# KrishnaswamyLab/graphtools

Hardware: NVIDIA B200
Metric: graph build points/sec (kernel+diff_op) (higher is better)
Workload: dtype f32 tensor-core select (f32 accumulate) / f64 values

## Files before the change

graphtools_b200/csrc/order.cu:

```cuda
#include "common.cuh"
#include "gtb200.h"

namespace {

constexpr int ORD_DMAX = 128;
constexpr int ORD_ASSIGN_THREADS = 128;
constexpr int ORD_CHUNK = 1024;
constexpr int LIST_UNITS = 8;

__global__ void __launch_bounds__(ORD_ASSIGN_THREADS) order_assign_kernel(const float* __restrict__ X, int64_t n, int d,
                                                                          int P, int64_t pstride,
                                                                          int32_t* __restrict__ cell) {
  extern __shared__ float4 piv4[];
  const int d4 = (d + 3) / 4;
  float* piv = reinterpret_cast<float*>(piv4);
  float* pn = piv + (size_t)P * d4 * 4;
  for (int i = threadIdx.x; i < P * d4 * 4; i += blockDim.x) {
    const int pv = i / (d4 * 4), k = i - pv * d4 * 4;
    piv[i] = k < d ? X[(int64_t)pv * pstride * d + k] : 0.f;
  }
  __syncthreads();
  for (int pv = threadIdx.x; pv < P; pv += blockDim.x) {
    float s = 0.f;
    for (int k = 0; k < d4 * 4; ++k) s = fmaf(piv[pv * d4 * 4 + k], piv[pv * d4 * 4 + k], s);
    pn[pv] = s;
  }
  __syncthreads();
  const int64_t r = (int64_t)blockIdx.x * blockDim.x + threadIdx.x;
  if (r >= n) return;
  float x[ORD_DMAX];
#pragma unroll
  for (int k = 0; k < ORD_DMAX; ++k) x[k] = k < d ? X[r * d + k] : 0.f;
  float best = gtb_inf_f();
  int bi = 0;
  for (int pv = 0; pv < P; ++pv) {
    const float4* pp = piv4 + pv * d4;
    float a0 = 0.f, a1 = 0.f;
#pragma unroll
    for (int k4 = 0; k4 < ORD_DMAX / 4; ++k4) {
      if (k4 < d4) {
        const float4 q = pp[k4];
        a0 = fmaf(x[4 * k4], q.x, a0);
        a1 = fmaf(x[4 * k4 + 1], q.y, a1);
        a0 = fmaf(x[4 * k4 + 2], q.z, a0);
        a1 = fmaf(x[4 * k4 + 3], q.w, a1);
      }
    }
    const float s = pn[pv] - 2.f * (a0 + a1);
    if (s < best) { best = s; bi = pv; }
  }
  cell[r] = bi;
}

__global__ void order_count_kernel(const int32_t* __restrict__ cell, int64_t n, int P, int32_t* __restrict__ counts) {
  extern __shared__ int32_t hist[];
  for (int p = threadIdx.x; p < P; p += blockDim.x) hist[p] = 0;
  __syncthreads();
  const int64_t r0 = (int64_t)blockIdx.x * ORD_CHUNK;
  for (int64_t r = r0 + threadIdx.x; r < n && r < r0 + ORD_CHUNK; r += blockDim.x) atomicAdd(&hist[cell[r]], 1);
  __syncthreads();
  for (int p = threadIdx.x; p < P; p += blockDim.x) counts[(int64_t)blockIdx.x * P + p] = hist[p];
}

__global__ void order_cellscan_kernel(int32_t* __restrict__ counts, int64_t nchunks, int P, int32_t* __restrict__ total) {
  const int lane = threadIdx.x & 31;
  const int p = (int)(((int64_t)blockIdx.x * blockDim.x + threadIdx.x) >> 5);
  if (p >= P) return;
  int run = 0;
  for (int64_t c0 = 0; c0 < nchunks; c0 += 32) {
    const int64_t c = c0 + lane;
    const int v = c < nchunks ? counts[c * P + p] : 0;
    int inc = v;
#pragma unroll
    for (int off = 1; off < 32; off <<= 1) {
      const int o = __shfl_up_sync(0xffffffffu, inc, off);
      if (lane >= off) inc += o;
    }
    if (c < nchunks) counts[c * P + p] = run + inc - v;
    run += __shfl_sync(0xffffffffu, inc, 31);
  }
  if (lane == 0) total[p] = run;
}

__global__ void __launch_bounds__(32) order_fill_kernel(const int32_t* __restrict__ cell, int64_t n, int P,
                                                        const int32_t* __restrict__ counts,
                                                        const int32_t* __restrict__ total, int32_t* __restrict__ perm) {
  extern __shared__ int64_t off[];
  const int lane = threadIdx.x;
  int64_t run = 0;
  for (int p0 = 0; p0 < P; p0 += 32) {
    const int p = p0 + lane;
    const int64_t v = p < P ? total[p] : 0;
    int64_t inc = v;
#pragma unroll
    for (int o = 1; o < 32; o <<= 1) {
      const int64_t u = __shfl_up_sync(0xffffffffu, inc, o);
      if (lane >= o) inc += u;
    }
    if (p < P) off[p] = run + inc - v + counts[(int64_t)blockIdx.x * P + p];
    run += __shfl_sync(0xffffffffu, inc, 31);
  }
  __syncwarp();
  const int64_t r0 = (int64_t)blockIdx.x * ORD_CHUNK;
  for (int64_t rb = r0; rb < n && rb < r0 + ORD_CHUNK; rb += 32) {
    const int64_t r = rb + lane;
    const bool ok = r < n;
    const int c = ok ? cell[r] : -1 - lane;
    const unsigned peers = __match_any_sync(0xffffffffu, c);
    const int rank = __popc(peers & ((1u << lane) - 1u));
    if (ok) perm[off[c] + rank] = (int32_t)r;
    __syncwarp();
    if (ok && rank == 0) off[c] += __popc(peers);
    __syncwarp();
  }
}

template <typename T>
__global__ void tile_geometry_kernel(const T* __restrict__ X, int64_t n, int d, const int32_t* __restrict__ perm,
                                     int64_t rows, int64_t ngroups, double* __restrict__ cent, double* __restrict__ rad) {
  constexpr int J = ORD_DMAX / 32;
  const int lane = threadIdx.x & 31;
  const int64_t g = ((int64_t)blockIdx.x * blockDim.x + threadIdx.x) >> 5;
  if (g >= ngroups) return;
  const int64_t r0 = g * rows, r1 = (r0 + rows < n) ? r0 + rows : n;
  double c[J];
#pragma unroll
  for (int j = 0; j < J; ++j) c[j] = 0.0;
#pragma unroll 8
  for (int64_t r = r0; r < r1; ++r) {
    const T* xr = X + (int64_t)perm[r] * d;
#pragma unroll
    for (int j = 0; j < J; ++j) {
      const int k = lane + 32 * j;
      if (k < d) c[j] += (double)xr[k];
    }
  }
  const double inv = r1 > r0 ? 1.0 / (double)(r1 - r0) : 0.0;
#pragma unroll
  for (int j = 0; j < J; ++j) c[j] *= inv;
  double m = 0.0;
#pragma unroll 8
  for (int64_t r = r0; r < r1; ++r) {
    const T* xr = X + (int64_t)perm[r] * d;
    double s = 0.0;
#pragma unroll
    for (int j = 0; j < J; ++j) {
      const int k = lane + 32 * j;
      if (k < d) {
        const double v = (double)xr[k] - c[j];
        s = fma(v, v, s);
      }
    }
#pragma unroll
    for (int o = 16; o > 0; o >>= 1) s += __shfl_xor_sync(0xffffffffu, s, o);
    m = fmax(m, s);
  }
#pragma unroll
  for (int j = 0; j < J; ++j) {
    const int k = lane + 32 * j;
    if (k < d) cent[(int64_t)k * ngroups + g] = c[j];
  }
  if (lane == 0) rad[g] = r1 > r0 ? __dsqrt_ru(m) : -1.0;
}

__global__ void tile_lists_count_kernel(const double* __restrict__ uc, const double* __restrict__ ur,
                                        const double* __restrict__ ub, int64_t nu, const double* __restrict__ rc,
                                        const double* __restrict__ rr, int64_t nt, int d, uint8_t* __restrict__ keep,
                                        int32_t* __restrict__ count) {
  __shared__ double cu[LIST_UNITS][ORD_DMAX];
  const int64_t u0 = (int64_t)blockIdx.y * LIST_UNITS;
  for (int i = threadIdx.x; i < LIST_UNITS * d; i += blockDim.x) {
    const int u = i / d, k = i - u * d;
    cu[u][k] = (u0 + u < nu) ? uc[(int64_t)k * nu + u0 + u] : 0.0;
  }
  __syncthreads();
  const int64_t t = (int64_t)blockIdx.x * blockDim.x + threadIdx.x;
  double s[LIST_UNITS];
#pragma unroll
  for (int u = 0; u < LIST_UNITS; ++u) s[u] = 0.0;
  if (t < nt) {
    for (int k = 0; k < d; ++k) {
      const double y = rc[(int64_t)k * nt + t];
#pragma unroll
      for (int u = 0; u < LIST_UNITS; ++u) {
        const double v = cu[u][k] - y;
        s[u] = fma(v, v, s[u]);
      }
    }
  }
  const double rt = t < nt ? rr[t] * (1.0 + 1e-12) : 0.0;
#pragma unroll
  for (int u = 0; u < LIST_UNITS; ++u) {
    const int64_t uu = u0 + u;
    bool k = false;
    if (t < nt && uu < nu && ur[uu] >= 0.0) {
      const double gap = sqrt(s[u]) * (1.0 - 1e-12) - ur[uu] * (1.0 + 1e-12) - rt;
      k = !(gap > 0.0 && gap * gap * (1.0 - 1e-12) >= ub[uu]);
    }
    if (t < nt && uu < nu) keep[uu * nt + t] = k ? 1 : 0;
    const unsigned b = __ballot_sync(0xffffffffu, k);
    if ((threadIdx.x & 31) == 0 && b) atomicAdd(&count[uu], __popc(b));
  }
}

__global__ void __launch_bounds__(256) tile_lists_fill_kernel(const uint8_t* __restrict__ keep, int64_t nt,
                                                              const int64_t* __restrict__ ptr,
                                                              int32_t* __restrict__ tiles) {
  __shared__ int wsum[8];
  const int64_t u = blockIdx.x;
  const int lane = threadIdx.x & 31, warp = threadIdx.x >> 5;
  int64_t run = ptr[u];
  for (int64_t t0 = 0; t0 < nt; t0 += 256) {
    const int64_t t = t0 + threadIdx.x;
    const bool k = t < nt && keep[u * nt + t];
    const unsigned b = __ballot_sync(0xffffffffu, k);
    if (lane == 0) wsum[warp] = __popc(b);
    __syncthreads();
    int before = 0, all = 0;
#pragma unroll
    for (int w = 0; w < 8; ++w) {
      before += (w < warp) ? wsum[w] : 0;
      all += wsum[w];
    }
    if (k) tiles[run + before + __popc(b & ((1u << lane) - 1u))] = (int32_t)t;
    run += all;
    __syncthreads();
  }
}

__global__ void unpermute_kernel(const int32_t* __restrict__ cand_p, const float* __restrict__ tau_p, int64_t nq, int S,
                                 int ntau, const int32_t* __restrict__ perm_q, const int32_t* __restrict__ perm_r,
                                 int32_t* __restrict__ cand, float* __restrict__ tau) {
  const int64_t e = (int64_t)blockIdx.x * blockDim.x + threadIdx.x;
  if (e >= nq * S) return;
  const int64_t i = e / S;
  const int s = (int)(e - i * S);
  const int64_t o = perm_q[i];
  const int32_t c = cand_p[e];
  cand[o * S + s] = c >= 0 ? perm_r[c] : c;
  if (s < ntau) tau[o * ntau + s] = tau_p[i * ntau + s];
}

}

extern "C" int gtb_order_assign(const float* X, int64_t n, int d, int P, int32_t* cell, void* stream) {
  GTB_CHECK_ARG(n > 0 && d > 0 && d <= ORD_DMAX, "bad shape (d <= 128)");
  GTB_CHECK_ARG(P >= 1 && P <= 512 && P <= n, "pivot count must be in [1, min(512, n)]");
  const size_t smem = ((size_t)P * ((d + 3) / 4) * 4 + P) * sizeof(float);
  GTB_CUDA(cudaFuncSetAttribute(order_assign_kernel, cudaFuncAttributeMaxDynamicSharedMemorySize, (int)smem));
  order_assign_kernel<<<(unsigned)gtb_cdiv(n, ORD_ASSIGN_THREADS), ORD_ASSIGN_THREADS, smem, (cudaStream_t)stream>>>(
      X, n, d, P, n / P, cell);
  GTB_CHECK_LAUNCH();
  return GTB_OK;
}

extern "C" int64_t gtb_order_ws_elems(int64_t n, int P) { return gtb_cdiv(n, ORD_CHUNK) * P + P; }

extern "C" int gtb_order_sort(const int32_t* cell, int64_t n, int P, int32_t* ws, int32_t* perm, void* stream) {
  GTB_CHECK_ARG(n > 0 && P >= 1 && P <= 512, "bad shape");
  cudaStream_t st = (cudaStream_t)stream;
  const int64_t nchunks = gtb_cdiv(n, ORD_CHUNK);
  int32_t* counts = ws;
  int32_t* total = ws + nchunks * P;
  order_count_kernel<<<(unsigned)nchunks, 256, P * sizeof(int32_t), st>>>(cell, n, P, counts);
  GTB_CHECK_LAUNCH();
  order_cellscan_kernel<<<(unsigned)gtb_cdiv(P, 8), 256, 0, st>>>(counts, nchunks, P, total);
  GTB_CHECK_LAUNCH();
  order_fill_kernel<<<(unsigned)nchunks, 32, P * sizeof(int64_t), st>>>(cell, n, P, counts, total, perm);
  GTB_CHECK_LAUNCH();
  return GTB_OK;
}

extern "C" int gtb_tile_geometry(const void* X, int64_t n, int d, int x64, const int32_t* perm, int64_t rows,
                                 int64_t ngroups, double* cent, double* rad, void* stream) {
  GTB_CHECK_ARG(n > 0 && d > 0 && d <= ORD_DMAX && rows > 0 && ngroups > 0, "bad shape (d <= 128)");
  const unsigned grid = (unsigned)gtb_cdiv(ngroups * 32, 256);
  if (x64)
    tile_geometry_kernel<double><<<grid, 256, 0, (cudaStream_t)stream>>>((const double*)X, n, d, perm, rows, ngroups,
                                                                         cent, rad);
  else
    tile_geometry_kernel<float><<<grid, 256, 0, (cudaStream_t)stream>>>((const float*)X, n, d, perm, rows, ngroups,
                                                                        cent, rad);
  GTB_CHECK_LAUNCH();
  return GTB_OK;
}

extern "C" int gtb_tile_lists_count(const double* uc, const double* ur, const double* ub, int64_t nu, const double* rc,
                                    const double* rr, int64_t nt, int d, uint8_t* keep, int32_t* count, void* stream) {
  GTB_CHECK_ARG(nu > 0 && nt > 0 && d > 0 && d <= ORD_DMAX, "bad shape (d <= 128)");
  GTB_CHECK_ARG(gtb_cdiv(nu, LIST_UNITS) < 65536, "too many units");
  cudaStream_t st = (cudaStream_t)stream;
  GTB_CUDA(cudaMemsetAsync(count, 0, nu * sizeof(int32_t), st));
  tile_lists_count_kernel<<<dim3((unsigned)gtb_cdiv(nt, 256), (unsigned)gtb_cdiv(nu, LIST_UNITS)), 256, 0, st>>>(
      uc, ur, ub, nu, rc, rr, nt, d, keep, count);
  GTB_CHECK_LAUNCH();
  return GTB_OK;
}

extern "C" int gtb_tile_lists_fill(const uint8_t* keep, int64_t nu, int64_t nt, const int64_t* ptr, int32_t* tiles,
                                   void* stream) {
  GTB_CHECK_ARG(nu > 0 && nt > 0, "bad shape");
  tile_lists_fill_kernel<<<(unsigned)nu, 256, 0, (cudaStream_t)stream>>>(keep, nt, ptr, tiles);
  GTB_CHECK_LAUNCH();
  return GTB_OK;
}

extern "C" int gtb_unpermute_candidates(const int32_t* cand_p, const float* tau_p, int64_t nq, int S, int ntau,
                                        const int32_t* perm_q, const int32_t* perm_r, int32_t* cand, float* tau,
                                        void* stream) {
  GTB_CHECK_ARG(nq > 0 && S > 0 && ntau >= 1 && ntau <= S, "bad shape");
  unpermute_kernel<<<(unsigned)gtb_cdiv(nq * S, 256), 256, 0, (cudaStream_t)stream>>>(cand_p, tau_p, nq, S, ntau,
                                                                                      perm_q, perm_r, cand, tau);
  GTB_CHECK_LAUNCH();
  return GTB_OK;
}
```

graphtools_b200/csrc/search_tc.cu:

```cuda
#include "common.cuh"
#include "gtb200.h"
#include "tc_ptx.cuh"
#include <cuda.h>
#include <cuda_bf16.h>
#include <cuda_fp16.h>

namespace {

#ifndef GTB_TC_CAP
#define GTB_TC_CAP 96
#endif
#ifndef GTB_TC_HYBRID
#define GTB_TC_HYBRID 4
#endif
constexpr int TC_M = 128, TC_N = 128, TC_CAP = GTB_TC_CAP, TC_S = 32, TC_GROUPS = 2, TC_THREADS = 64 + 128 * TC_GROUPS;
static_assert(TC_CAP % 32 == 0 && TC_CAP >= TC_S + 64 && TC_CAP <= 128, "candidate buffer: TC_S kept + two batches of 32");
constexpr float TC_BIG = 1e29f;
constexpr float TC_PAD_NORM = 1e30f;
constexpr float TC_BIG_H = 50000.f;
constexpr float TC_PAD_NORM_H = 60000.f;
constexpr float TC_H_MAXNORM = 8192.f;
constexpr int64_t TC_SPLIT_ROWS_MAX = 40 * 4 * 128;
#ifndef GTB_TC_SEED_K
#define GTB_TC_SEED_K 8
#endif
constexpr int TC_SEED_K = GTB_TC_SEED_K;

using namespace gtbptx;

struct TcParams {
  int64_t nq, nq_pad, nr, nr_pad;
  int nks;
  int64_t nrounds;
  int64_t n_qclusters, tiles_per_split;
  unsigned int* sync_ctr;
  int64_t tile_stride;
  const float* seed_tau;
  int64_t q_unit0, split_k, split_row0, split_rows;
  uint2* piece_buf; uint2* piece_meta;
  const int64_t* unit_ptr; const int32_t* unit_tiles; const int32_t* unit_order; int64_t n_units;
  const float* qn2;
  int32_t* cand_idx; uint2* cand_buf; float* tau;
  const float* lim2; int2* pairs; unsigned long long capacity; unsigned long long* counter; int32_t* rowcnt;
};

__device__ __forceinline__ uint32_t f2ord(uint32_t bits) {
  return bits ^ ((uint32_t)((int32_t)bits >> 31) | 0x80000000u);
}
__device__ __forceinline__ float ord2f(uint32_t u) {
  return __uint_as_float((u & 0x80000000u) ? (u ^ 0x80000000u) : ~u);
}

template <int LS, int CAP>
__device__ __noinline__ float compact_row(uint2* buf, int cnt, int lane) {
  constexpr int NSLOT = CAP / 32;
  constexpr unsigned long long NONE = ~0ull;
  uint2 t[NSLOT];
  unsigned long long key[NSLOT];
#pragma unroll
  for (int i = 0; i < NSLOT; ++i) {
    const int e = i * 32 + lane;
    t[i] = make_uint2(0u, 0u);
    key[i] = NONE;
    if (e < cnt) {
      t[i] = buf[e];
      key[i] = ((unsigned long long)f2ord(t[i].x) << 32) | (unsigned long long)t[i].y;
    }
  }
  unsigned long long lo = 0ull, hi = NONE, T = NONE;
  for (int iter = 0; iter < CAP + 1; ++iter) {
    unsigned m[NSLOT];
#pragma unroll
    for (int i = 0; i < NSLOT; ++i) m[i] = __ballot_sync(0xffffffffu, key[i] > lo && key[i] < hi);
    unsigned long long cand = 0ull;
    unsigned mm = 0u;
#pragma unroll
    for (int i = 0; i < NSLOT; ++i) {
      const int sl = (i + iter) % NSLOT;
      unsigned long long ks = key[0];
      unsigned ms = m[0];
#pragma unroll
      for (int q = 1; q < NSLOT; ++q) { if (sl == q) { ks = key[q]; ms = m[q]; } }
      if (mm == 0u && ms != 0u) { cand = ks; mm = ms; }
    }
    if (mm == 0u) break;
    const int src = (iter & 2) ? (31 - __clz(mm)) : (__ffs(mm) - 1);
    const unsigned long long pv = __shfl_sync(0xffffffffu, cand, src);
    int c = 0;
#pragma unroll
    for (int i = 0; i < NSLOT; ++i) c += __popc(__ballot_sync(0xffffffffu, key[i] < pv));
    if (c == LS - 1) { T = pv; break; }
    if (c >= LS) hi = pv; else lo = pv;
  }
  int base = 0;
  const unsigned lt = (1u << lane) - 1u;
#pragma unroll
  for (int i = 0; i < NSLOT; ++i) {
    const bool keep = key[i] <= T;
    const unsigned km = __ballot_sync(0xffffffffu, keep);
    if (keep) buf[base + __popc(km & lt)] = t[i];
    base += __popc(km);
  }
  return ord2f((uint32_t)(T >> 32));
}

__device__ __forceinline__ float tmin32(const uint32_t (&r)[32]) {
  float b[11];
#pragma unroll
  for (int i = 0; i < 10; ++i)
    b[i] = fminf(fminf(__uint_as_float(r[3 * i]), __uint_as_float(r[3 * i + 1])), __uint_as_float(r[3 * i + 2]));
  b[10] = fminf(__uint_as_float(r[30]), __uint_as_float(r[31]));
  const float c0 = fminf(fminf(b[0], b[1]), b[2]), c1 = fminf(fminf(b[3], b[4]), b[5]);
  const float c2 = fminf(fminf(b[6], b[7]), b[8]), c3 = fminf(b[9], b[10]);
  return fminf(fminf(fminf(c0, c1), c2), c3);
}

constexpr int TC_SYNC_EVERY = 128;

__device__ __forceinline__ void tmem_st8(uint32_t taddr, const float4& a, const float4& b) {
  asm volatile("tcgen05.st.sync.aligned.32x32b.x8.b32 [%0], {%1, %2, %3, %4, %5, %6, %7, %8};"
               ::"r"(taddr), "r"(__float_as_uint(a.x)), "r"(__float_as_uint(a.y)), "r"(__float_as_uint(a.z)),
               "r"(__float_as_uint(a.w)), "r"(__float_as_uint(b.x)), "r"(__float_as_uint(b.y)),
               "r"(__float_as_uint(b.z)), "r"(__float_as_uint(b.w))
               : "memory");
}
__device__ __forceinline__ void tc_mma_ts_pred(bool bf16, uint32_t d_tmem, uint32_t a_tmem, uint64_t bdesc,
                                               uint32_t idesc, uint32_t accumulate, uint32_t leader) {
  if (bf16) {
    asm volatile(
        "{\n .reg .pred p, q;\n setp.ne.b32 p, %4, 0;\n setp.ne.b32 q, %5, 0;\n"
        " @q tcgen05.mma.cta_group::1.kind::f16 [%0], [%1], %2, %3, p;\n}"
        ::"r"(d_tmem), "r"(a_tmem), "l"(bdesc), "r"(idesc), "r"(accumulate), "r"(leader)
        : "memory");
  } else {
    asm volatile(
        "{\n .reg .pred p, q;\n setp.ne.b32 p, %4, 0;\n setp.ne.b32 q, %5, 0;\n"
        " @q tcgen05.mma.cta_group::1.kind::tf32 [%0], [%1], %2, %3, p;\n}"
        ::"r"(d_tmem), "r"(a_tmem), "l"(bdesc), "r"(idesc), "r"(accumulate), "r"(leader)
        : "memory");
  }
}
__device__ __forceinline__ void tc_commit_pred(uint32_t bar, uint32_t leader) {
  asm volatile(
      "{\n .reg .pred q;\n setp.ne.b32 q, %1, 0;\n"
      " @q tcgen05.commit.cta_group::1.mbarrier::arrive::one.shared::cluster.b64 [%0];\n}"
      ::"r"(bar), "r"(leader)
      : "memory");
}
__device__ __forceinline__ void tc_commit_mc_pred(uint32_t bar, uint16_t mask, uint32_t leader) {
  asm volatile(
      "{\n .reg .pred q;\n setp.ne.b32 q, %2, 0;\n"
      " @q tcgen05.commit.cta_group::1.mbarrier::arrive::one.shared::cluster.multicast::cluster.b64 [%0], %1;\n}"
      ::"r"(bar), "h"(mask), "r"(leader)
      : "memory");
}

template <int MODE, int CL, int FMT, int LS, int QT, bool PIECE = false, bool WIDE = false,
          bool LISTED = false>
__global__ void __launch_bounds__(TC_THREADS, 1)
search_tc_kernel(const __grid_constant__ CUtensorMap mBh, const __grid_constant__ CUtensorMap mBht,
                 const __grid_constant__ CUtensorMap mBl, const __grid_constant__ CUtensorMap mBlt,
                 const void* __restrict__ q_hi_v, const void* __restrict__ q_lo_v, TcParams p) {
  extern __shared__ unsigned char smem_raw[];
  const uint32_t raw = smem_u32(smem_raw);
  const uint32_t base = (raw + 1023u) & ~1023u;
  unsigned char* gbase = smem_raw + (base - raw);

  constexpr bool BF16 = FMT != 0;
  constexpr int NPROD = (FMT == 3) ? 1 : (FMT == 2) ? 2 : 3;
  constexpr int NPART = (FMT == 3) ? 1 : 2;
  constexpr float BIG = (FMT >= 2) ? TC_BIG_H : TC_BIG;
  constexpr int EPK = BF16 ? 16 : 8;
  static_assert(QT == 1 || (QT == 2 && FMT >= 2 && MODE != 1), "two query tiles per CTA: fp16 top-k / seed only");
  static_assert(MODE != 2 || (FMT == 3 && QT == 2), "seed sweeps use the one-product flavour");
  static_assert(FMT != 3 || QT == 2, "the one-product flavour runs two query tiles per CTA");
  static_assert(!WIDE || (FMT == 2 && QT == 1 && !PIECE), "wide operand rows: fp16x2, one query tile per CTA");
  static_assert(!LISTED || (MODE == 0 && FMT == 3 && !PIECE && !WIDE), "tile lists: one-product top-k sweep");
  constexpr int LSO = (QT == 2) ? 2 * LS : LS;
  constexpr int CAP = (LSO > 32) ? TC_GROUPS * TC_CAP : TC_CAP;
  static_assert(CAP >= LSO + 64, "room for a list and two batches of 32");
  constexpr bool HYB = !(FMT == 3 && LS == 32);
  const int nks = p.nks;
  const int nfull = nks / 4, ntail = nks % 4;
  const int a_lo_col = nks * 8;
  const int nch = WIDE ? (nks + 7) / 8 : 1;
  const uint32_t sizeB = (uint32_t)TC_N * (WIDE ? 8 : nks) * 32;
  const char* q_hi = reinterpret_cast<const char*>(q_hi_v);
  const char* q_lo = reinterpret_cast<const char*>(q_lo_v);
  constexpr int NS = BF16 ? (NPART == 1 ? 4 : 3) : 2;
  constexpr int NA = (BF16 && !WIDE) ? 3 : 2;
  constexpr int ACC0 = (BF16 && !WIDE) ? 128 : 256;
  const uint32_t B0 = base;
  const uint32_t bar0 = B0 + NPART * NS * sizeB;
  const uint32_t bar_a = bar0, full_b = bar0 + 8, empty_b = bar0 + 40, tm_full = bar0 + 72, tm_empty = bar0 + 104;
  const uint32_t round_done = bar0 + 136;
  uint32_t* tmem_slot = reinterpret_cast<uint32_t*>(gbase + (bar0 - base) + 144);

  const int warp = threadIdx.x >> 5, lane = threadIdx.x & 31;
  const int64_t n_clusters = gridDim.x / CL;
  const int64_t cluster_id = blockIdx.x / CL;
  const int64_t nrounds = p.nrounds;
  const int64_t qcluster = cluster_id % p.n_qclusters;
  const int64_t tile0 = (cluster_id / p.n_qclusters) * p.tiles_per_split;
  const int64_t tstride = (MODE != 1) ? p.tile_stride : 1;
  const int64_t tiles_left = (p.nr_pad / TC_N + tstride - 1) / tstride - tile0;
  const int64_t ntiles = tiles_left < p.tiles_per_split ? tiles_left : p.tiles_per_split;
  auto unit_of = [&](int64_t round) -> int64_t {
    const int64_t slot = round * n_clusters + ((round & 1) ? (n_clusters - 1 - qcluster) : qcluster);
    return slot < p.n_units ? (int64_t)p.unit_order[slot] : slot;
  };
  auto list_lo = [&](int64_t u) -> int64_t { return u < p.n_units ? p.unit_ptr[u] : 0; };
  auto list_len = [&](int64_t u) -> int64_t { return u < p.n_units ? p.unit_ptr[u + 1] - p.unit_ptr[u] : 0; };
  auto q0_of = [&](int64_t round, int qt) {
    const int64_t u = LISTED ? unit_of(round) : (PIECE ? p.q_unit0 : 0) + qcluster + round * n_clusters;
    return ((u * CL + (blockIdx.x % CL)) * QT + qt) * TC_M;
  };
  static_assert(!PIECE || (MODE == 0 && FMT == 3), "piece launches belong to the one-product top-k sweep");
  auto btile = [&](int64_t round, int64_t t) { return (tile0 + ((round & 1) ? (ntiles - 1 - t) : t)) * tstride; };
  const uint32_t crank = (CL > 1) ? cluster_ctarank() : 0u;
  constexpr uint16_t cmask = (uint16_t)((1u << CL) - 1u);
  constexpr int ROWS = TC_N / CL;

  if (threadIdx.x == 0) {
    mbar_init(bar_a, 4 * QT);
    mbar_init(round_done, 1);
    for (int s = 0; s < NS; ++s) {
      mbar_init(full_b + 8 * s, 1);
      mbar_init(empty_b + 8 * s, CL);
    }
    for (int s = 0; s < NA; ++s) {
      mbar_init(tm_full + 8 * s, 1);
      mbar_init(tm_empty + 8 * s, 4);
    }
    asm volatile("fence.mbarrier_init.release.cluster;" ::: "memory");
    asm volatile("fence.proxy.async.shared::cta;" ::: "memory");
  }
  if (warp == 1) {
    asm volatile("tcgen05.alloc.cta_group::1.sync.aligned.shared::cta.b32 [%0], %1;" ::"r"(smem_u32(tmem_slot)),
                 "r"(512));
    asm volatile("tcgen05.relinquish_alloc_permit.cta_group::1.sync.aligned;" ::);
  }
  tc_fence_before();
  __syncthreads();
  if (CL > 1) cluster_sync_all();
  tc_fence_after();
  const uint32_t tmem_base = *tmem_slot;

  if (warp == 0 && WIDE) {
    if (lane == 0) {
      int64_t it = 0, sit = 0;
      for (int64_t round = 0; round < nrounds; ++round) {
        for (int64_t t = 0; t < ntiles; ++t, ++it) {
          if (p.sync_ctr != nullptr && (it % TC_SYNC_EVERY) == 0) {
            const unsigned int target = (unsigned int)(it / TC_SYNC_EVERY + 1) * gridDim.x;
            atomicAdd(p.sync_ctr, 1u);
            for (int polls = 0; polls < (1 << 16); ++polls) {
              unsigned int seen;
              asm volatile("ld.acquire.gpu.global.u32 %0, [%1];" : "=r"(seen) : "l"(p.sync_ctr) : "memory");
              if (seen >= target) break;
              __nanosleep(64);
            }
          }
          const int row0 = (int)(btile(round, t) * TC_N) + (int)crank * ROWS;
          for (int c = 0; c < nch; ++c, ++sit) {
            const int s = (int)(sit % NS);
            const uint32_t ph = (uint32_t)((sit / NS) & 1);
            const int nk = (nks - 8 * c) < 8 ? (nks - 8 * c) : 8;
            const int nf = nk / 4, nt2 = nk % 4;
            mbar_wait(empty_b + 8 * s, ph ^ 1);
            mbar_arrive_expect_tx(full_b + 8 * s, (uint32_t)(NPART * TC_N * nk * 32));
            for (int part = 0; part < NPART; ++part) {
              const CUtensorMap* mm = part ? &mBl : &mBh;
              const CUtensorMap* mt = part ? &mBlt : &mBht;
              const uint32_t dst = B0 + (NPART * s + part) * sizeB;
              for (int b = 0; b < nf; ++b) {
                const uint32_t d = dst + b * (TC_N * 128) + crank * (ROWS * 128);
                if (CL > 1) tma_load_2d_mc(d, mm, full_b + 8 * s, (c * 8 + b * 4) * EPK, row0, cmask);
                else tma_load_2d(d, mm, full_b + 8 * s, (c * 8 + b * 4) * EPK, row0);
              }
              for (int t2 = 0; t2 < nt2; ++t2) {
                const uint32_t d = dst + nf * (TC_N * 128) + t2 * (TC_N * 32) + crank * (ROWS * 32);
                if (CL > 1) tma_load_2d_mc(d, mt, full_b + 8 * s, (c * 8 + nf * 4 + t2) * EPK, row0, cmask);
                else tma_load_2d(d, mt, full_b + 8 * s, (c * 8 + nf * 4 + t2) * EPK, row0);
              }
            }
          }
        }
      }
    }
  } else if (warp == 1 && WIDE) {
    const bool leader = elect_one();
    const uint32_t lead = leader ? 1u : 0u;
    constexpr uint32_t fmt = (FMT == 0) ? 2u : (FMT == 1 ? 1u : 0u);
    const uint32_t idesc = (1u << 4) | (fmt << 7) | (fmt << 10) | ((uint32_t)(TC_N >> 3) << 17) |
                           ((uint32_t)(TC_M >> 4) << 24);
    const uint64_t bd_main0 = make_desc(B0, 1024, 2);
    const uint32_t part_off = sizeB >> 4, stage_off = (NPART * sizeB) >> 4;
    int64_t it = 0, sit = 0;
    for (int64_t round = 0; round < nrounds; ++round) {
      mbar_wait(bar_a, (uint32_t)(round & 1));
      tc_fence_after();
      for (int64_t tile = 0; tile < ntiles; ++tile, ++it) {
        const int ac_i = (int)(it % NA);
        const uint32_t aph = (uint32_t)((it / NA) & 1);
        mbar_wait(tm_empty + 8 * ac_i, aph ^ 1);
        tc_fence_after();
        const uint32_t d_tmem = tmem_base + (uint32_t)(ACC0 + ac_i * TC_N);
        uint32_t accum = 0;
#pragma unroll 1
        for (int c = 0; c < nch; ++c, ++sit) {
          const int s = (int)(sit % NS);
          const uint32_t ph = (uint32_t)((sit / NS) & 1);
          const int nk = (nks - 8 * c) < 8 ? (nks - 8 * c) : 8;
          const int nf = nk / 4, nt2 = nk % 4;
          mbar_wait(full_b + 8 * s, ph);
          tc_fence_after();
          const uint64_t bd_tail0 = make_desc(B0 + nf * (TC_N * 128), 256, 6);
#pragma unroll 1
          for (int prod = 0; prod < NPROD; ++prod) {
            uint32_t ac = tmem_base + (uint32_t)(c * 64);
            const uint64_t boff = (uint64_t)(s * stage_off + ((prod == 1) ? part_off : 0u));
            uint64_t bd = bd_main0 + boff;
#pragma unroll 1
            for (int blk = 0; blk < nf; ++blk) {
#pragma unroll
              for (int sub = 0; sub < 4; ++sub) {
                tc_mma_ts_pred(BF16, d_tmem, ac + sub * 8, bd + sub * 2, idesc, accum, lead);
                accum = 1;
              }
              bd += (TC_N * 128) >> 4;
              ac += 32;
            }
            bd = bd_tail0 + boff;
#pragma unroll 1
            for (int t = 0; t < nt2; ++t) {
              tc_mma_ts_pred(BF16, d_tmem, ac, bd, idesc, accum, lead);
              accum = 1;
              bd += (TC_N * 32) >> 4;
              ac += 8;
            }
          }
          if (CL > 1) tc_commit_mc_pred(empty_b + 8 * s, cmask, lead);
          else tc_commit_pred(empty_b + 8 * s, lead);
        }
        tc_commit_pred(tm_full + 8 * ac_i, lead);
      }
      tc_commit_pred(round_done, lead);
    }
  } else if (warp == 0) {
    if (lane == 0) {
      int64_t it = 0;
      for (int64_t round = 0; round < nrounds; ++round) {
        int64_t nt = ntiles, lo = 0;
        if (LISTED) { const int64_t u = unit_of(round); lo = list_lo(u); nt = list_len(u); }
        for (int64_t t = 0; t < nt; ++t, ++it) {
          const int s = (int)(it % NS);
          const uint32_t ph = (uint32_t)((it / NS) & 1);
          if (p.sync_ctr != nullptr && (it % TC_SYNC_EVERY) == 0) {
            const unsigned int target = (unsigned int)(it / TC_SYNC_EVERY + 1) * gridDim.x;
            atomicAdd(p.sync_ctr, 1u);
            for (int polls = 0; polls < (1 << 16); ++polls) {
              unsigned int seen;
              asm volatile("ld.acquire.gpu.global.u32 %0, [%1];" : "=r"(seen) : "l"(p.sync_ctr) : "memory");
              if (seen >= target) break;
              __nanosleep(64);
            }
          }
          mbar_wait(empty_b + 8 * s, ph ^ 1);
          mbar_arrive_expect_tx(full_b + 8 * s, NPART * sizeB);
          const int64_t tile = LISTED ? (int64_t)p.unit_tiles[lo + t] : btile(round, t);
          const int row0 = (int)(tile * TC_N) + (int)crank * ROWS;
          for (int part = 0; part < NPART; ++part) {
            const CUtensorMap* mm = part ? &mBl : &mBh;
            const CUtensorMap* mt = part ? &mBlt : &mBht;
            const uint32_t dst = B0 + (NPART * s + part) * sizeB;
            for (int b = 0; b < nfull; ++b) {
              const uint32_t d = dst + b * (TC_N * 128) + crank * (ROWS * 128);
              if (CL > 1) tma_load_2d_mc(d, mm, full_b + 8 * s, b * 4 * EPK, row0, cmask);
              else tma_load_2d(d, mm, full_b + 8 * s, b * 4 * EPK, row0);
            }
            for (int t2 = 0; t2 < ntail; ++t2) {
              const uint32_t d = dst + nfull * (TC_N * 128) + t2 * (TC_N * 32) + crank * (ROWS * 32);
              if (CL > 1) tma_load_2d_mc(d, mt, full_b + 8 * s, (nfull * 4 + t2) * EPK, row0, cmask);
              else tma_load_2d(d, mt, full_b + 8 * s, (nfull * 4 + t2) * EPK, row0);
            }
          }
        }
      }
    }
  } else if (warp == 1) {
    const bool leader = elect_one();
    constexpr uint32_t fmt = (FMT == 0) ? 2u : (FMT == 1 ? 1u : 0u);
    const uint32_t idesc = (1u << 4) | (fmt << 7) | (fmt << 10) | ((uint32_t)(TC_N >> 3) << 17) |
                           ((uint32_t)(TC_M >> 4) << 24);
    const uint64_t bd_main0 = make_desc(B0, 1024, 2);
    const uint64_t bd_tail0 = make_desc(B0 + nfull * (TC_N * 128), 256, 6);
    const uint32_t part_off = sizeB >> 4, stage_off = (NPART * sizeB) >> 4;
    int64_t it = 0;
    for (int64_t round = 0; round < nrounds; ++round) {
    mbar_wait(bar_a, (uint32_t)(round & 1));
    tc_fence_after();
    const int64_t nt = LISTED ? list_len(unit_of(round)) : ntiles;
    for (int64_t tile = 0; tile < nt; ++tile, ++it) {
      const int s = (int)(it % NS);
      const uint32_t ph = (uint32_t)((it / NS) & 1);
      mbar_wait(full_b + 8 * s, ph);
      const uint32_t lead = leader ? 1u : 0u;
#pragma unroll 1
      for (int qt = 0; qt < QT; ++qt) {
      const int64_t ait = it * QT + qt;
      const int ac_i = (int)(ait % NA);
      const uint32_t aph = (uint32_t)((ait / NA) & 1);
      mbar_wait(tm_empty + 8 * ac_i, aph ^ 1);
      tc_fence_after();
      const uint32_t d_tmem = tmem_base + (uint32_t)(ACC0 + ac_i * TC_N);
      uint32_t accum = 0;
#pragma unroll 1
      for (int prod = 0; prod < NPROD; ++prod) {
        uint32_t ac = tmem_base + (uint32_t)((prod == 2) ? a_lo_col : 0) + (uint32_t)(qt * 64);
        const uint64_t boff = (uint64_t)(s * stage_off + ((prod == 1) ? part_off : 0u));
        uint64_t bd = bd_main0 + boff;
#pragma unroll 1
        for (int blk = 0; blk < nfull; ++blk) {
#pragma unroll
          for (int sub = 0; sub < 4; ++sub) {
            tc_mma_ts_pred(BF16, d_tmem, ac + sub * 8, bd + sub * 2, idesc, accum, lead);
            accum = 1;
          }
          bd += (TC_N * 128) >> 4;
          ac += 32;
        }
        bd = bd_tail0 + boff;
#pragma unroll 1
        for (int t = 0; t < ntail; ++t) {
          tc_mma_ts_pred(BF16, d_tmem, ac, bd, idesc, accum, lead);
          accum = 1;
          bd += (TC_N * 32) >> 4;
          ac += 8;
        }
      }
      tc_commit_pred(tm_full + 8 * ac_i, lead);
      }
      if (CL > 1) tc_commit_mc_pred(empty_b + 8 * s, cmask, lead);
      else tc_commit_pred(empty_b + 8 * s, lead);
    }
    tc_commit_pred(round_done, leader ? 1u : 0u);
    }
  } else {
    const int quad = warp & 3;
    const int grp = (warp - 2) >> 2;
    float* xpose = reinterpret_cast<float*>(gbase + (bar0 - base) + 256) + (warp - 2) * 32;
    const int row = quad * 32 + lane;
    const uint32_t lane_addr = tmem_base + ((uint32_t)(quad * 32) << 16);
    const int my_qt = (QT == 2) ? grp : 0;
    const int lgrp = (QT == 2) ? 0 : grp;
    const uint32_t a_col0 = (uint32_t)(my_qt * 64);
    int64_t it_run = 0;
    for (int64_t round = 0; round < nrounds; ++round) {
    int64_t nt = ntiles, lo = 0;
    if (LISTED) { const int64_t u = unit_of(round); lo = list_lo(u); nt = list_len(u); }
    const int64_t q0 = q0_of(round, my_qt);
    const int64_t gq = q0 + row;
    const bool valid = gq < p.nq;

    if (grp == 0 || QT == 2) {
      if (round > 0) { mbar_wait(round_done, (uint32_t)((round - 1) & 1)); tc_fence_after(); }
      const bool in_pad = gq < p.nq_pad;
      const float4* rh = reinterpret_cast<const float4*>(q_hi + (in_pad ? gq : 0) * (int64_t)(nks * 32));
      const float4* rl = reinterpret_cast<const float4*>(q_lo + (in_pad ? gq : 0) * (int64_t)(nks * 32));
      const float4 z4 = make_float4(0.f, 0.f, 0.f, 0.f);
      for (int ks = 0; ks < nks; ++ks) {
        tmem_st8(lane_addr + a_col0 + (uint32_t)(ks * 8), in_pad ? rh[2 * ks] : z4, in_pad ? rh[2 * ks + 1] : z4);
        if (NPROD == 3)
          tmem_st8(lane_addr + (uint32_t)(a_lo_col + ks * 8), in_pad ? rl[2 * ks] : z4, in_pad ? rl[2 * ks + 1] : z4);
      }
      asm volatile("tcgen05.wait::st.sync.aligned;" ::: "memory");
      tc_fence_before();
      __syncwarp();
      if (lane == 0) mbar_arrive(bar_a);
    }

    const float nx = valid ? p.qn2[gq] : 0.f;
    float thr;
    if (MODE == 0) {
      thr = valid ? BIG : -gtb_inf_f();
      if (valid && p.seed_tau != nullptr) {
        const float t0 = p.seed_tau[gq * TC_GROUPS] - nx;
        if (t0 < BIG) thr = t0;
      }
    } else if (MODE == 1) {
      thr = valid ? fminf(p.lim2[gq] - nx, BIG) : -gtb_inf_f();
    } else {
      thr = 0.f;
    }
    float best[TC_SEED_K];
#pragma unroll
    for (int i = 0; i < TC_SEED_K; ++i) best[i] = BIG;
    int cnt = 0;
    const int64_t boff = valid ? (gq * TC_GROUPS + lgrp) * TC_CAP : 0;
    uint2* wbuf = p.cand_buf + (q0 + quad * 32) * TC_GROUPS * TC_CAP;
    uint2* mybuf = p.cand_buf + boff;
    if (PIECE) {
      uint2* pb = p.piece_buf + ((cluster_id / p.n_qclusters) * p.split_rows - p.split_row0) * (TC_GROUPS * TC_CAP);
      wbuf = pb + (q0 + quad * 32) * TC_GROUPS * TC_CAP;
      mybuf = pb + boff;
    }

    const int64_t it0 = LISTED ? it_run : round * ntiles;
    if (LISTED) it_run += nt;
    for (int64_t t = (QT == 2) ? 0 : ((grp + (it0 & 1)) & 1); t < nt; t += (QT == 2 ? 1 : TC_GROUPS)) {
      const int64_t it = it0 + t;
      const int64_t tile = LISTED ? (int64_t)p.unit_tiles[lo + t] : btile(round, t);
      const int64_t ait = (QT == 2) ? (it * 2 + grp) : it;
      const int s = (int)(ait % NA);
      const uint32_t ph = (uint32_t)((ait / NA) & 1);
      mbar_wait(tm_full + 8 * s, ph);
      tc_fence_after();
      uint32_t r0[32], r1[32], r2[32], r3[32];
      __syncwarp();
      const uint32_t acc_addr = lane_addr + (uint32_t)(ACC0 + s * TC_N);
      tmem_ld32_nowait(acc_addr, r0);
      tmem_ld32_nowait(acc_addr + 32, r1);
      tmem_ld32_nowait(acc_addr + 64, r2);
      tmem_ld32_nowait(acc_addr + 96, r3);
      tmem_wait_ld(r0, r1, r2, r3);
      tc_fence_before();
      __syncwarp();
      if (lane == 0) mbar_arrive(tm_empty + 8 * s);
#ifdef GTB_EXP_NOSELECT
      continue;
#endif
      if (MODE == 2) {
        float v = fminf(fminf(tmin32(r0), tmin32(r1)), fminf(tmin32(r2), tmin32(r3)));
#pragma unroll
        for (int i = 0; i < TC_SEED_K; ++i) {
          const float lo = fminf(best[i], v);
          v = fmaxf(best[i], v);
          best[i] = lo;
        }
        continue;
      }
      const float bm0 = tmin32(r0), bm1 = tmin32(r1), bm2 = tmin32(r2), bm3 = tmin32(r3);
      unsigned h0 = __ballot_sync(0xffffffffu, (MODE == 0) ? (bm0 < thr) : (bm0 <= thr));
      unsigned h1 = __ballot_sync(0xffffffffu, (MODE == 0) ? (bm1 < thr) : (bm1 <= thr));
      unsigned h2 = __ballot_sync(0xffffffffu, (MODE == 0) ? (bm2 < thr) : (bm2 <= thr));
      unsigned h3 = __ballot_sync(0xffffffffu, (MODE == 0) ? (bm3 < thr) : (bm3 <= thr));
#ifdef GTB_EXP_NOSERVICE
      h0 = h1 = h2 = h3 = 0;
#endif
      if ((h0 | h1 | h2 | h3) == 0u) continue;
#pragma unroll
      for (int part = 0; part < TC_N / 32; ++part) {
        unsigned hot = part == 0 ? h0 : part == 1 ? h1 : part == 2 ? h2 : h3;
        if (hot == 0u) continue;
        float v[32];
#pragma unroll
        for (int j = 0; j < 32; ++j)
          v[j] = __uint_as_float(part == 0 ? r0[j] : part == 1 ? r1[j] : part == 2 ? r2[j] : r3[j]);
        const int32_t col0 = (int32_t)(tile * TC_N) + part * 32;
        if (MODE == 0) {
#if GTB_TC_HYBRID > 0
          if (HYB && __popc(hot) >= GTB_TC_HYBRID) {
            uint2* wp = mybuf + cnt;
#pragma unroll
            for (int j = 0; j < 32; ++j) {
              asm volatile(
                  "{\n .reg .pred p;\n setp.lt.f32 p, %1, %2;\n @p st.global.v2.b32 [%0], {%3, %4};\n"
                  " @p add.u64 %0, %0, 8;\n}"
                  : "+l"(wp)
                  : "f"(v[j]), "f"(thr), "r"(__float_as_uint(v[j])), "r"(col0 + j)
                  : "memory");
            }
            cnt = (int)(wp - mybuf);
            hot = 0;
          }
#endif
        }
        while (hot) {
          const int L = __ffs(hot) - 1;
          hot &= hot - 1;
          if (lane == L) {
            float4* dst4 = reinterpret_cast<float4*>(xpose);
#pragma unroll
            for (int j = 0; j < 8; ++j) dst4[j] = make_float4(v[4 * j], v[4 * j + 1], v[4 * j + 2], v[4 * j + 3]);
          }
          __syncwarp();
          const float x = xpose[lane];
          const float tL = __shfl_sync(0xffffffffu, thr, L);
          const bool pass = (MODE == 0) ? (x < tL) : (x <= tL);
          const unsigned pm = __ballot_sync(0xffffffffu, pass);
          const int npass = __popc(pm);
          const int rank = __popc(pm & ((1u << lane) - 1u));
          if (MODE == 0) {
            const int cL = __shfl_sync(0xffffffffu, cnt, L);
            if (pass) wbuf[(L * TC_GROUPS + lgrp) * TC_CAP + cL + rank] = make_uint2(__float_as_uint(x), (uint32_t)(col0 + lane));
            if (lane == L) cnt += npass;
          } else {
            unsigned long long basepos = 0;
            if (lane == L) {
              basepos = atomicAdd(p.counter, (unsigned long long)npass);
              atomicAdd(p.rowcnt + gq, npass);
            }
            basepos = __shfl_sync(0xffffffffu, basepos, L);
            if (pass && basepos + (unsigned long long)rank < p.capacity)
              p.pairs[basepos + rank] = make_int2((int)(q0 + quad * 32 + L), col0 + lane);
          }
          __syncwarp();
        }
        if (MODE == 0) {
          unsigned need = __ballot_sync(0xffffffffu, cnt > CAP - 32);
          while (need) {
            const int owner = __ffs(need) - 1;
            need &= need - 1;
            const int ocnt = __shfl_sync(0xffffffffu, cnt, owner);
            __syncwarp();
            const float nt = compact_row<LSO, CAP>(wbuf + (owner * TC_GROUPS + lgrp) * TC_CAP, ocnt, lane);
            __syncwarp();
            if (lane == owner) { thr = nt; cnt = LSO; }
          }
        }
      }
    }

    if (MODE == 2) {
      if (valid) {
        const float tv = (best[TC_SEED_K - 1] >= BIG) ? gtb_inf_f() : best[TC_SEED_K - 1] + nx;
        p.tau[gq * TC_GROUPS] = tv;
        p.tau[gq * TC_GROUPS + 1] = tv;
      }
    }
    if (MODE == 0) {
      unsigned need = __ballot_sync(0xffffffffu, cnt > LSO);
      while (need) {
        const int owner = __ffs(need) - 1;
        need &= need - 1;
        const int ocnt = __shfl_sync(0xffffffffu, cnt, owner);
        __syncwarp();
        const float nt = compact_row<LSO, CAP>(wbuf + (owner * TC_GROUPS + lgrp) * TC_CAP, ocnt, lane);
        __syncwarp();
        if (lane == owner) { thr = nt; cnt = LSO; }
      }
      __syncwarp();
      if (valid) {
        const float tv = (thr >= BIG) ? gtb_inf_f() : thr + nx;
        if (PIECE) {
          p.piece_meta[(cluster_id / p.n_qclusters) * p.split_rows + (gq - p.split_row0)] =
              make_uint2((uint32_t)cnt, __float_as_uint(tv));
        } else {
          int32_t* out = p.cand_idx + gq * (TC_GROUPS * LS) + lgrp * LS;
          for (int e = 0; e < LSO; ++e) out[e] = (e < cnt) ? (int32_t)p.cand_buf[boff + e].y : -1;
          p.tau[gq * TC_GROUPS + lgrp] = tv;
          if (QT == 2) p.tau[gq * TC_GROUPS + 1] = tv;
        }
      }
    }
    }
  }

  tc_fence_before();
  __syncthreads();
  if (warp == 1) {
    tc_fence_after();
    asm volatile("tcgen05.dealloc.cta_group::1.sync.aligned.b32 %0, %1;" ::"r"(tmem_base), "r"(512));
  }
  if (CL > 1) cluster_sync_all();
}

constexpr int TC_SPLIT_MAX = 4, TC_MERGE_WARPS = 4;

template <int LS>
__global__ void __launch_bounds__(TC_MERGE_WARPS * 32) merge_pieces_kernel(TcParams p) {
  constexpr int CAP = TC_GROUPS * TC_CAP, MCAP = TC_SPLIT_MAX * LS;
  __shared__ uint2 stage_s[TC_MERGE_WARPS][MCAP];
  const int lane = threadIdx.x & 31, warp = threadIdx.x >> 5;
  const int64_t r = (int64_t)blockIdx.x * TC_MERGE_WARPS + warp;
  const int64_t gq = p.split_row0 + r;
  if (r >= p.split_rows || gq >= p.nq) return;
  uint2* stage = stage_s[warp];
  const float nx = p.qn2[gq];
  float tau = gtb_inf_f();
  int total = 0;
  for (int pc = 0; pc < (int)p.split_k; ++pc) {
    const uint2 meta = p.piece_meta[pc * p.split_rows + r];
    const int c = (int)meta.x < LS ? (int)meta.x : LS;
    tau = fminf(tau, __uint_as_float(meta.y));
    const uint2* src = p.piece_buf + (pc * p.split_rows + r) * CAP;
    for (int e = lane; e < c; e += 32) stage[total + e] = src[e];
    total += c;
  }
  __syncwarp();
  if (total > LS) {
    const float t = compact_row<LS, MCAP>(stage, total, lane);
    tau = fminf(tau, t + nx);
    total = LS;
    __syncwarp();
  }
  int32_t* out = p.cand_idx + gq * LS;
  for (int e = lane; e < LS; e += 32) out[e] = (e < total) ? (int32_t)stage[e].y : -1;
  if (lane == 0) { p.tau[gq * TC_GROUPS] = tau; p.tau[gq * TC_GROUPS + 1] = tau; }
}

__device__ __forceinline__ float to_tf32(float x) {
  uint32_t r;
  asm("cvt.rna.tf32.f32 %0, %1;" : "=r"(r) : "f"(x));
  return __uint_as_float(r);
}

__global__ void tc_norms_kernel(const float* __restrict__ X, int64_t n, int d, const float* __restrict__ mean,
                                int64_t n_pad, float* __restrict__ norm2, float* __restrict__ maxnorm) {
  const int lane = threadIdx.x & 31;
  const int64_t r = ((int64_t)blockIdx.x * blockDim.x + threadIdx.x) >> 5;
  if (r >= n_pad) return;
  float out = 0.f;
  if (r < n) {
    double s = 0.0;
    for (int k = lane; k < d; k += 32) {
      double v = (double)(X[r * d + k] - (mean ? mean[k] : 0.f));
      s += v * v;
    }
#pragma unroll
    for (int off = 16; off > 0; off >>= 1) s += __shfl_xor_sync(0xffffffffu, s, off);
    out = __double2float_ru(s);
  }
  if (lane == 0) {
    norm2[r] = (r < n) ? out : TC_PAD_NORM;
    if (maxnorm && r < n) atomicMax((int*)maxnorm, __float_as_int(out));
  }
}

__global__ void tc_split_kernel(const float* __restrict__ X, int64_t n, int d, const float* __restrict__ mean,
                                int role, const float* __restrict__ norm2, int64_t n_pad, int Kp,
                                float* __restrict__ hi, float* __restrict__ lo) {
  const int64_t e = (int64_t)blockIdx.x * blockDim.x + threadIdx.x;
  if (e >= n_pad * Kp) return;
  const int64_t r = e / Kp;
  const int k = (int)(e - r * Kp);
  float v = 0.f;
  if (r < n) {
    if (k < d) {
      v = X[r * d + k] - (mean ? mean[k] : 0.f);
      if (role == 1) v *= -2.f;
    } else if (k == d) {
      v = (role == 1) ? norm2[r] : 1.f;
    }
  } else if (role == 1 && k == d) {
    v = TC_PAD_NORM;
  }
  const float h = to_tf32(v);
  hi[e] = h;
  lo[e] = to_tf32(v - h);
}

__global__ void tc_split16_kernel(const float* __restrict__ X, int64_t n, int d, const float* __restrict__ mean,
                                  int role, const float* __restrict__ norm2, int64_t n_pad, int Kp,
                                  __nv_bfloat16* __restrict__ hi, __nv_bfloat16* __restrict__ lo) {
  const int64_t e = (int64_t)blockIdx.x * blockDim.x + threadIdx.x;
  if (e >= n_pad * Kp) return;
  const int64_t r = e / Kp;
  const int k = (int)(e - r * Kp);
  float v = 0.f;
  if (r < n) {
    if (k < d) {
      v = X[r * d + k] - (mean ? mean[k] : 0.f);
      if (role == 1) v *= -2.f;
    } else if (k == d) {
      v = (role == 1) ? norm2[r] : 1.f;
    }
  } else if (role == 1 && k == d) {
    v = TC_PAD_NORM;
  }
  const __nv_bfloat16 h = __float2bfloat16_rn(v);
  hi[e] = h;
  lo[e] = __float2bfloat16_rn(v - __bfloat162float(h));
}

__global__ void tc_split16h_kernel(const float* __restrict__ X, int64_t n, int d, const float* __restrict__ mean,
                                   int role, const float* __restrict__ norm2, int64_t n_pad, int Kp, float scale,
                                   __half* __restrict__ hi, __half* __restrict__ lo) {
  const int64_t e = (int64_t)blockIdx.x * blockDim.x + threadIdx.x;
  if (e >= n_pad * Kp) return;
  const int64_t r = e / Kp;
  const int k = (int)(e - r * Kp);
  float v = 0.f;
  if (r < n) {
    if (k < d) {
      v = (X[r * d + k] - (mean ? mean[k] : 0.f)) * scale;
      if (role == 1) v *= -2.f;
    } else if (k == d) {
      v = (role == 1) ? norm2[r] * scale * scale : 1.f;
    } else if (k == d + 1) {
      if (role == 1) {
        const float nv = norm2[r] * scale * scale;
        v = nv - __half2float(__float2half_rn(nv));
      } else {
        v = 1.f;
      }
    }
  } else if (role == 1 && k == d) {
    v = TC_PAD_NORM_H;
  }
  const __half h = __float2half_rn(v);
  hi[e] = h;
  lo[e] = (k >= d) ? __float2half_rn(0.f) : __float2half_rn(v - __half2float(h));
}

int make_map(CUtensorMap* m, const void* ptr, int64_t rows, int Kp, int box_k, int box_rows, bool sw128, int fmt) {
  const bool bf16 = fmt != 0;
  EncodeTiledFn enc = get_encode();
  if (!enc) { gtb_set_error("cuTensorMapEncodeTiled entry point not available"); return GTB_ERR_CUDA; }
  cuuint64_t dims[2] = {(cuuint64_t)Kp, (cuuint64_t)rows};
  cuuint64_t strides[1] = {(cuuint64_t)Kp * (bf16 ? 2 : 4)};
  cuuint32_t box[2] = {(cuuint32_t)box_k, (cuuint32_t)box_rows};
  cuuint32_t estr[2] = {1, 1};
  CUresult r = enc(m, fmt == 1 ? CU_TENSOR_MAP_DATA_TYPE_BFLOAT16 : (fmt >= 2 ? CU_TENSOR_MAP_DATA_TYPE_FLOAT16 : CU_TENSOR_MAP_DATA_TYPE_FLOAT32), 2, (void*)ptr, dims, strides, box, estr,
                   CU_TENSOR_MAP_INTERLEAVE_NONE, sw128 ? CU_TENSOR_MAP_SWIZZLE_128B : CU_TENSOR_MAP_SWIZZLE_32B,
                   CU_TENSOR_MAP_L2_PROMOTION_L2_256B, CU_TENSOR_MAP_FLOAT_OOB_FILL_NONE);
  if (r != CUDA_SUCCESS) { gtb_set_error("cuTensorMapEncodeTiled failed (%d)", (int)r); return GTB_ERR_CUDA; }
  return GTB_OK;
}

template <int MODE, int CL, int FMT, int LS, int QT = 1, bool WIDE = false>
int launch_tc_cl(const void* q_hi, const void* q_lo, const void* r_hi, const void* r_lo, int Kp, TcParams& p,
                 cudaStream_t st) {
  CUtensorMap mBh, mBht, mBl, mBlt;
  int rc;
  constexpr bool BF16 = FMT != 0;
  constexpr int EPK = BF16 ? 16 : 8;
  p.nks = Kp / EPK;
  if ((rc = make_map(&mBh, r_hi, p.nr_pad, Kp, 4 * EPK, TC_N / CL, true, FMT))) return rc;
  if ((rc = make_map(&mBht, r_hi, p.nr_pad, Kp, EPK, TC_N / CL, false, FMT))) return rc;
  if ((rc = make_map(&mBl, r_lo, p.nr_pad, Kp, 4 * EPK, TC_N / CL, true, FMT))) return rc;
  if ((rc = make_map(&mBlt, r_lo, p.nr_pad, Kp, EPK, TC_N / CL, false, FMT))) return rc;
  constexpr int NPART = (FMT == 3) ? 1 : 2;
  constexpr int NS = BF16 ? (NPART == 1 ? 4 : 3) : 2;
  size_t smem = 1024 + (size_t)NPART * NS * TC_N * (WIDE ? 8 : p.nks) * 32 + 256 + 1024;
  auto kern = search_tc_kernel<MODE, CL, FMT, LS, QT, false, WIDE>;
  GTB_CUDA(cudaFuncSetAttribute(kern, cudaFuncAttributeMaxDynamicSharedMemorySize, (int)smem));
  int dev = 0, nsm = 0;
  GTB_CUDA(cudaGetDevice(&dev));
  GTB_CUDA(cudaDeviceGetAttribute(&nsm, cudaDevAttrMultiProcessorCount, dev));
  const int64_t n_cluster_tiles = gtb_cdiv(p.nq_pad / TC_M, CL * QT);
  int64_t n_clusters = n_cluster_tiles < (nsm / CL) ? n_cluster_tiles : (nsm / CL);
  p.nrounds = gtb_cdiv(n_cluster_tiles, n_clusters);
  if (p.tile_stride < 1 || MODE == 1) p.tile_stride = 1;
  const int64_t total_tiles = gtb_cdiv(p.nr_pad / TC_N, p.tile_stride);
  p.n_qclusters = n_clusters;
  p.tiles_per_split = total_tiles;
  int64_t splits = 1;
  if (MODE == 1 && n_cluster_tiles * 2 <= nsm / CL && total_tiles >= 16) {
    splits = (nsm / CL) / n_cluster_tiles;
    if (splits > total_tiles / 8) splits = total_tiles / 8;
    p.tiles_per_split = gtb_cdiv(total_tiles, splits);
    splits = gtb_cdiv(total_tiles, p.tiles_per_split);
// ... 275 lines not shown
```

Measured before the change: 12.52 million.

## Register-tile pivot assignment and defer tile-list load in listed sweep

The pivot assignment kernel is rewritten as a register-blocked tile: each block stages 128 rows and 32-pivot chunks in shared memory, and each thread accumulates a 4x8 row-by-pivot block. Per-warp best results are then merged through shared memory. This replaces the one-row-per-thread loop that kept a 128-float row in registers and read every pivot from shared memory. In the listed tensor-core sweep, the hybrid predicated-store path is enabled, and the unit_tiles global load is deferred until a hit is found.

```diff
diff --git a/graphtools_b200/csrc/order.cu b/graphtools_b200/csrc/order.cu
--- a/graphtools_b200/csrc/order.cu
+++ b/graphtools_b200/csrc/order.cu
@@ -4,52 +4,96 @@
 namespace {
 
 constexpr int ORD_DMAX = 128;
-constexpr int ORD_ASSIGN_THREADS = 128;
 constexpr int ORD_CHUNK = 1024;
 constexpr int LIST_UNITS = 8;
+constexpr int ORD_AROWS = 128, ORD_APIV = 32, ORD_AR = 4, ORD_AP = 8, ORD_ASSIGN_THREADS = 128;
 
 __global__ void __launch_bounds__(ORD_ASSIGN_THREADS) order_assign_kernel(const float* __restrict__ X, int64_t n, int d,
                                                                           int P, int64_t pstride,
                                                                           int32_t* __restrict__ cell) {
-  extern __shared__ float4 piv4[];
+  extern __shared__ float4 sm4[];
   const int d4 = (d + 3) / 4;
-  float* piv = reinterpret_cast<float*>(piv4);
-  float* pn = piv + (size_t)P * d4 * 4;
-  for (int i = threadIdx.x; i < P * d4 * 4; i += blockDim.x) {
-    const int pv = i / (d4 * 4), k = i - pv * d4 * 4;
-    piv[i] = k < d ? X[(int64_t)pv * pstride * d + k] : 0.f;
-  }
+  const int rs4 = d4 | 1;
+  float4* xs = sm4;
+  float4* ps = sm4 + ORD_AROWS * rs4;
+  float* pn = reinterpret_cast<float*>(ps + ORD_APIV * d4);
+  __shared__ float bv[ORD_ASSIGN_THREADS / 32][ORD_AROWS];
+  __shared__ int bp[ORD_ASSIGN_THREADS / 32][ORD_AROWS];
+  const int lane = threadIdx.x & 31, warp = threadIdx.x >> 5;
+  const int64_t r0 = (int64_t)blockIdx.x * ORD_AROWS;
+  for (int i = threadIdx.x; i < ORD_AROWS * d4 * 4; i += blockDim.x) {
+    const int rr = i / (d4 * 4), k = i - rr * d4 * 4;
+    reinterpret_cast<float*>(xs + rr * rs4)[k] = (k < d && r0 + rr < n) ? X[(r0 + rr) * d + k] : 0.f;
+  }
+  float best[ORD_AR];
+  int bi[ORD_AR];
+#pragma unroll
+  for (int i = 0; i < ORD_AR; ++i) { best[i] = gtb_inf_f(); bi[i] = 0; }
+  for (int p0 = 0; p0 < P; p0 += ORD_APIV) {
+    __syncthreads();
+    for (int i = threadIdx.x; i < ORD_APIV * d4 * 4; i += blockDim.x) {
+      const int pv = i / (d4 * 4), k = i - pv * d4 * 4;
+      reinterpret_cast<float*>(ps)[i] = (k < d && p0 + pv < P) ? X[(int64_t)(p0 + pv) * pstride * d + k] : 0.f;
+    }
+    __syncthreads();
+    if (threadIdx.x < ORD_APIV) {
+      const float* pp = reinterpret_cast<const float*>(ps + threadIdx.x * d4);
+      float s = 0.f;
+      for (int k = 0; k < d4 * 4; ++k) s = fmaf(pp[k], pp[k], s);
+      pn[threadIdx.x] = s;
+    }
+    __syncthreads();
+    float a0[ORD_AR][ORD_AP], a1[ORD_AR][ORD_AP];
+#pragma unroll
+    for (int i = 0; i < ORD_AR; ++i)
+#pragma unroll
+      for (int j = 0; j < ORD_AP; ++j) { a0[i][j] = 0.f; a1[i][j] = 0.f; }
+    const float4* xr = xs + lane * rs4;
+    const float4* pw = ps + warp * ORD_AP * d4;
+#pragma unroll 2
+    for (int k4 = 0; k4 < d4; ++k4) {
+      float4 x[ORD_AR];
+#pragma unroll
+      for (int i = 0; i < ORD_AR; ++i) x[i] = xr[i * 32 * rs4 + k4];
+#pragma unroll
+      for (int j = 0; j < ORD_AP; ++j) {
+        const float4 q = pw[j * d4 + k4];
+#pragma unroll
+        for (int i = 0; i < ORD_AR; ++i) {
+          a0[i][j] = fmaf(x[i].x, q.x, a0[i][j]);
+          a1[i][j] = fmaf(x[i].y, q.y, a1[i][j]);
+          a0[i][j] = fmaf(x[i].z, q.z, a0[i][j]);
+          a1[i][j] = fmaf(x[i].w, q.w, a1[i][j]);
+        }
+      }
+    }
+#pragma unroll
+    for (int j = 0; j < ORD_AP; ++j) {
+      const int pv = p0 + warp * ORD_AP + j;
+      if (pv < P) {
+#pragma unroll
+        for (int i = 0; i < ORD_AR; ++i) {
+          const float s = pn[warp * ORD_AP + j] - 2.f * (a0[i][j] + a1[i][j]);
+          if (s < best[i]) { best[i] = s; bi[i] = pv; }
+        }
+      }
+    }
+  }
+#pragma unroll
+  for (int i = 0; i < ORD_AR; ++i) { bv[warp][lane + 32 * i] = best[i]; bp[warp][lane + 32 * i] = bi[i]; }
   __syncthreads();
-  for (int pv = threadIdx.x; pv < P; pv += blockDim.x) {
-    float s = 0.f;
-    for (int k = 0; k < d4 * 4; ++k) s = fmaf(piv[pv * d4 * 4 + k], piv[pv * d4 * 4 + k], s);
-    pn[pv] = s;
-  }
-  __syncthreads();
-  const int64_t r = (int64_t)blockIdx.x * blockDim.x + threadIdx.x;
-  if (r >= n) return;
-  float x[ORD_DMAX];
-#pragma unroll
-  for (int k = 0; k < ORD_DMAX; ++k) x[k] = k < d ? X[r * d + k] : 0.f;
-  float best = gtb_inf_f();
-  int bi = 0;
-  for (int pv = 0; pv < P; ++pv) {
-    const float4* pp = piv4 + pv * d4;
-    float a0 = 0.f, a1 = 0.f;
-#pragma unroll
-    for (int k4 = 0; k4 < ORD_DMAX / 4; ++k4) {
-      if (k4 < d4) {
-        const float4 q = pp[k4];
-        a0 = fmaf(x[4 * k4], q.x, a0);
-        a1 = fmaf(x[4 * k4 + 1], q.y, a1);
-        a0 = fmaf(x[4 * k4 + 2], q.z, a0);
-        a1 = fmaf(x[4 * k4 + 3], q.w, a1);
-      }
-    }
-    const float s = pn[pv] - 2.f * (a0 + a1);
-    if (s < best) { best = s; bi = pv; }
-  }
-  cell[r] = bi;
+  const int rr = threadIdx.x;
+  if (r0 + rr < n) {
+    float b = bv[0][rr];
+    int c = bp[0][rr];
+#pragma unroll
+    for (int w = 1; w < ORD_ASSIGN_THREADS / 32; ++w) {
+      const float v = bv[w][rr];
+      const int pw2 = bp[w][rr];
+      if (v < b || (v == b && pw2 < c)) { b = v; c = pw2; }
+    }
+    cell[r0 + rr] = c;
+  }
 }
 
 __global__ void order_count_kernel(const int32_t* __restrict__ cell, int64_t n, int P, int32_t* __restrict__ counts) {
@@ -246,9 +290,10 @@
 extern "C" int gtb_order_assign(const float* X, int64_t n, int d, int P, int32_t* cell, void* stream) {
   GTB_CHECK_ARG(n > 0 && d > 0 && d <= ORD_DMAX, "bad shape (d <= 128)");
   GTB_CHECK_ARG(P >= 1 && P <= 512 && P <= n, "pivot count must be in [1, min(512, n)]");
-  const size_t smem = ((size_t)P * ((d + 3) / 4) * 4 + P) * sizeof(float);
+  const int d4 = (d + 3) / 4;
+  const size_t smem = (size_t)(ORD_AROWS * (d4 | 1) + ORD_APIV * d4) * sizeof(float4) + ORD_APIV * sizeof(float);
   GTB_CUDA(cudaFuncSetAttribute(order_assign_kernel, cudaFuncAttributeMaxDynamicSharedMemorySize, (int)smem));
-  order_assign_kernel<<<(unsigned)gtb_cdiv(n, ORD_ASSIGN_THREADS), ORD_ASSIGN_THREADS, smem, (cudaStream_t)stream>>>(
+  order_assign_kernel<<<(unsigned)gtb_cdiv(n, ORD_AROWS), ORD_ASSIGN_THREADS, smem, (cudaStream_t)stream>>>(
       X, n, d, P, n / P, cell);
   GTB_CHECK_LAUNCH();
   return GTB_OK;
diff --git a/graphtools_b200/csrc/search_tc.cu b/graphtools_b200/csrc/search_tc.cu
--- a/graphtools_b200/csrc/search_tc.cu
+++ b/graphtools_b200/csrc/search_tc.cu
@@ -179,7 +179,7 @@
   constexpr int LSO = (QT == 2) ? 2 * LS : LS;
   constexpr int CAP = (LSO > 32) ? TC_GROUPS * TC_CAP : TC_CAP;
   static_assert(CAP >= LSO + 64, "room for a list and two batches of 32");
-  constexpr bool HYB = !(FMT == 3 && LS == 32);
+  constexpr bool HYB = !(FMT == 3 && LS == 32) || LISTED;
   const int nks = p.nks;
   const int nfull = nks / 4, ntail = nks % 4;
   const int a_lo_col = nks * 8;
@@ -510,7 +510,7 @@
     if (LISTED) it_run += nt;
     for (int64_t t = (QT == 2) ? 0 : ((grp + (it0 & 1)) & 1); t < nt; t += (QT == 2 ? 1 : TC_GROUPS)) {
       const int64_t it = it0 + t;
-      const int64_t tile = LISTED ? (int64_t)p.unit_tiles[lo + t] : btile(round, t);
+      const int64_t tile_t = LISTED ? 0 : btile(round, t);
       const int64_t ait = (QT == 2) ? (it * 2 + grp) : it;
       const int s = (int)(ait % NA);
       const uint32_t ph = (uint32_t)((ait / NA) & 1);
@@ -549,6 +549,7 @@
       h0 = h1 = h2 = h3 = 0;
 #endif
       if ((h0 | h1 | h2 | h3) == 0u) continue;
+      const int64_t tile = LISTED ? (int64_t)p.unit_tiles[lo + t] : tile_t;
 #pragma unroll
       for (int part = 0; part < TC_N / 32; ++part) {
         unsigned hot = part == 0 ? h0 : part == 1 ? h1 : part == 2 ? h2 : h3;
```

Result: faster. 14.52 million (median of 6 runs) (+16.0%).
